# daviidsilvaa/MPI-Model

Hardware: AMD Instinct MI355X
Metric: cell-updates/s (GCUPS) per step + % of HBM roofline (higher is better)
Workload: dtype f64; 1 GPU; c3: 32768x32768 fp64 global, row slabs (BASELINE configs[2]); ranks=1, rows_per_gpu=32768, n_attr=1, parallelism=row-slab x1, rows_per_wave=2548

## Files before the change

mpi-model_amd/csrc/mm_engine.hip:

```cpp
#include <rccl/rccl.h>

#include <algorithm>
#include <cmath>
#include <cstdio>
#include <cstdlib>
#include <cstring>
#include <map>
#include <string>
#include <vector>

#include "../../include/mpimodel.h"
#include "mm_inst.hpp"
#include "mm_plan.hpp"

static_assert(MM_FIELD_MAX_STEPS == mm::kFieldMaxSteps, "include/mpimodel.h: MM_FIELD_MAX_STEPS");

namespace {

thread_local std::string g_last_error;

int fail(int code, const std::string& msg) {
    g_last_error = msg;
    return code;
}
// ... 212 lines not shown
}

constexpr int kPermIdentity = 0 | 1 << 2 | 2 << 4 | 3 << 6;

int relabel(const mm_engine* e, mm::PassArgs& A) {
    if (e->na == 1) return kPermIdentity;
    const Pass& p = e->passes[0];
    int perm[mm::kMaxAttr], inv[mm::kMaxAttr], n = 0;
    for (int a = 0; a < e->na; ++a)
        if ((p.diffuse_mask >> a) & 1) perm[n++] = a;
    const int nd = n;
    for (int a = 0; a < e->na; ++a)
        if (!((p.diffuse_mask >> a) & 1)) perm[n++] = a;
    int code = 0;
    for (int i = 0; i < e->na; ++i) {
        inv[perm[i]] = i;
        code |= perm[i] << (2 * i);
        A.in[i] = e->buf[e->cur][perm[i]];
        A.out[i] = e->buf[e->cur ^ 1][perm[i]];
        A.drate[i] = p.drate[perm[i]];
    }
    A.diffuse_mask = (1 << nd) - 1;
    for (size_t t = 0; t < p.pre.size(); ++t) {
        A.pre_a[t] = (signed char)inv[p.pre[t].a];
        A.pre_b[t] = (signed char)(p.pre[t].b < 0 ? -1 : inv[p.pre[t].b]);
    }
    for (size_t t = 0; t < p.post.size(); ++t) {
        A.post_a[t] = (signed char)inv[p.post[t].a];
        A.post_b[t] = (signed char)(p.post[t].b < 0 ? -1 : inv[p.post[t].b]);
    }
    return code;
}

int slots_per_cu(mm_engine* e, mm::Kernel kernel, int k, bool red) {
    const bool wide = kernel == mm::kWide;
    const mm::KernelInst* inst = mm::find_inst(
        inst_key(e, kernel, k, wide ? (e->na > 1 ? 2 : 4) : 2, true, red, e->variant & 1));
    if (!inst) return 1;
    int& s = e->slots[inst];
    if (!s) s = std::max(1, mm::inst_blocks_per_cu(*inst) * (wide ? 1 : mm::kWavesPerBlock));
    return s;
}

bool field_halo(const mm_engine* e) { return e->d.nranks > 1 || e->d.halo_mode != MM_HALO_NONE; }

void sync_program(mm_engine* e) {
    mm::PlanIn& pin = e->pin;
    pin.n_passes = (int)e->passes.size();
    const Pass* p = pin.n_passes == 1 ? &e->passes[0] : nullptr;
    pin.diffuse_mask = p ? p->diffuse_mask : 0;
    pin.chains = p && !(p->pre.empty() && p->post.empty());
    pin.ring = wring(e);
    pin.field = false;
    for (const Pass& q : e->passes) pin.field = pin.field || q.field_mask != 0;
    bool eight = e->na > 1;
    for (const Pass& q : e->passes)
        eight = eight || !q.pre.empty() || !q.post.empty() || q.field_mask != 0;
    pin.knobs.th = eight ? 8 : e->th_env;
    const bool alone = e->na == 1 && p && p->field_mask == 1 && p->diffuse_mask == 0 && !pin.chains;
    pin.field_k = alone ? mm::field_k_for(pin, field_halo(e)) : 0;
}

int halo_rccl(mm_engine* e, int depth) {
    const int r = e->d.rank, n = e->d.nranks;
    const long long P = e->pitch, h = e->d.h;
    const size_t cnt = (size_t)(depth * P);
    MM_NCCL(ncclGroupStart());
    for (int a = 0; a < e->na; ++a) {
        double* b = e->buf[e->cur][a];
        if (e->self_halo) {
// ... 29 lines not shown
    if (rccl_halo(e)) MM_TRY(halo_rccl(e, depth));
    MM_HIP(hipStreamWaitEvent(e->s_comm, e->ev_comp_mark, 0));
    return MM_OK;
}

int unsplit_halo(mm_engine* e, int depth) {
    if (!rccl_halo(e)) return MM_OK;
    MM_HIP(hipEventRecord(e->ev_ready, e->s_comp));
    MM_HIP(hipStreamWaitEvent(e->s_comm, e->ev_ready, 0));
    MM_TRY(halo_rccl(e, depth));
    MM_HIP(hipEventRecord(e->ev_halo, e->s_comm));
    MM_HIP(hipStreamWaitEvent(e->s_comp, e->ev_halo, 0));
    return MM_OK;
}

int launch(mm_engine* e, const mm::PassLaunches& pl, bool red, const mm::PassArgs& A, hipStream_t s,
           bool border) {
    const int nt = border ? 0 : e->variant;
    if (pl.kern.kernel != mm::kOneStep)
        MM_HIP(mm::launch_kstep(
            inst_key(e, pl.kern.kernel, pl.depth, pl.kern.cols, A.seg != 0, red, nt & 1), A, s));
    else if (A.field_mask)
        MM_HIP(mm::launch_field(e->na, red, A, s, nt));
    else
        MM_HIP(mm::launch_pass(e->na, red, A, s, e->variant));
    return MM_OK;
}

void set_launch(mm::PassArgs& A, const mm::Launch& l) {
    A.ra0 = (int)l.lo, A.ra1 = (int)l.hi, A.rb0 = (int)l.lo2, A.rb1 = (int)l.hi2;
    A.seg = l.seg, A.th = l.th, A.th_edge = l.th_edge, A.xcd_remap = l.xcd_remap;
    A.nstrips = l.nstrips;
    A.waves_a = l.waves_a, A.waves_total = l.waves_total, A.partial_base = l.partial_base;
}

int enqueue_pass(mm_engine* e, const Pass& p, int k, int mask, bool time_it, bool prime = false) {
    const bool red = mask != 0;
    const mm::PassLaunches pl = mm::pass_launches(e->pin, k, red);
    mm::PassArgs A;
    fill_args(e, p, A);
    const int perm = pl.kern.kernel == mm::kWide ? relabel(e, A) : kPermIdentity;
    mm::PassArgs B = A;
    set_launch(A, pl.interior);
    set_launch(B, pl.border);
    if (prime) {
        A.waves_total = B.waves_total = 0;
        A.waves_a = B.waves_a = -1;
        MM_TRY(launch(e, pl, red, A, e->s_comp, false));
        if (pl.split) MM_TRY(launch(e, pl, red, B, e->s_comm, true));
        return MM_OK;
    }
    if (pl.split)
        MM_TRY(split_comp(e));
    else if (e->pin.split)
        MM_TRY(unsplit_halo(e, pl.depth));
    hipEvent_t t0 = nullptr, t1 = nullptr;
    if (time_it) {
        t0 = next_event(e);
        t1 = next_event(e);
        if (!t0 || !t1) return fail(MM_ERR_HIP, "hipEventCreate failed");
        e->ev_bytes.resize(e->ev_used / 2);
        e->ev_bytes.back() = (16.0 * e->na + 8.0 * __builtin_popcount((unsigned)p.field_mask)) *
                             (double)(pl.interior.hi - pl.interior.lo) * (double)e->d.W;
        MM_HIP(hipEventRecord(t0, e->s_comp));
    }
    MM_TRY(launch(e, pl, red, A, e->s_comp, false));
// ... 215 lines not shown
}

int mm_engine_create(const mm_desc* desc, mm_engine** out) {
    if (!desc || !out) return fail(MM_ERR_INVALID, "mm_engine_create: null argument");
    *out = nullptr;
    const mm_desc& d = *desc;
    if (d.H <= 0 || d.W <= 0 || d.h <= 0 || d.x_init < 0 || d.x_init + d.h > d.H)
        return fail(MM_ERR_INVALID, "mm_engine_create: slab outside the grid");
    if (d.n_attr < 1 || d.n_attr > mm::kMaxAttr)
        return fail(MM_ERR_INVALID, "mm_engine_create: n_attr must be 1..4");
    if (d.nranks < 1 || d.rank < 0 || d.rank >= d.nranks)
        return fail(MM_ERR_INVALID, "mm_engine_create: bad rank/nranks");
    if (d.nranks == 1 && (d.x_init != 0 || d.h != d.H))
        return fail(MM_ERR_INVALID, "mm_engine_create: a single slab must own the whole grid");
    if (d.halo_mode == MM_HALO_RCCL && !d.comm_id)
        return fail(MM_ERR_INVALID, "mm_engine_create: MM_HALO_RCCL needs comm_id");
    if (d.nranks > 1 && d.halo_mode == MM_HALO_NONE)
        return fail(MM_ERR_INVALID, "mm_engine_create: nranks > 1 needs a halo mode");
    if (d.W > (1LL << 30) || d.h > (1LL << 30))
        return fail(MM_ERR_INVALID, "mm_engine_create: slab too large");

    mm_engine* e = new mm_engine();
    e->d = d;
    e->na = d.n_attr;
    e->pitch = (d.W + mm::kStripCols - 1) / mm::kStripCols * mm::kStripCols;
    e->rows_alloc = d.h + 2 * mm::kGhost;
    mm::PlanIn& pin = e->pin;
    pin.H = d.H, pin.W = d.W, pin.h = d.h, pin.x_init = d.x_init, pin.nranks = d.nranks;
    pin.pitch = e->pitch, pin.n_attr = d.n_attr;
    pin.min_rows = std::min<long long>(d.h, d.H / d.nranks);
    pin.knobs = mm::read_knobs([](const char* name) -> const char* { return std::getenv(name); });
    e->th_env = pin.knobs.th;
    pin.slots = [e](mm::Kernel kernel, int k, bool red) { return slots_per_cu(e, kernel, k, red); };
    e->variant = mm::kernel_variant(pin);

    auto cleanup = [&](int rc) {
        mm_engine_destroy(e);
        return rc;
    };
    hipError_t he = hipSetDevice(d.device);
    if (he != hipSuccess) return cleanup(fail(MM_ERR_HIP, std::string("hipSetDevice: ") + hipGetErrorString(he)));
    he = hipDeviceGetAttribute(&e->pin.ncu, hipDeviceAttributeMultiprocessorCount, d.device);
    if (he != hipSuccess || e->pin.ncu <= 0) e->pin.ncu = 256;

    const size_t per = (size_t)e->rows_alloc * (size_t)e->pitch;
    const size_t per_al = (per + 31) / 32 * 32;
    e->bytes = sizeof(double) * per_al * 2 * (size_t)e->na;
    if (hipStreamCreateWithFlags(&e->s_comp, hipStreamNonBlocking) != hipSuccess ||
        hipStreamCreateWithFlags(&e->s_comm, hipStreamNonBlocking) != hipSuccess ||
        hipEventCreateWithFlags(&e->ev_ready, hipEventDisableTiming) != hipSuccess ||
        hipEventCreateWithFlags(&e->ev_halo, hipEventDisableTiming) != hipSuccess ||
        hipEventCreateWithFlags(&e->ev_comp_mark, hipEventDisableTiming) != hipSuccess ||
        hipEventCreateWithFlags(&e->ev_comm_done, hipEventDisableTiming) != hipSuccess)
        return cleanup(fail(MM_ERR_HIP, "stream/event creation failed"));

    he = hipMalloc(&e->base, e->bytes);
    if (he != hipSuccess) return cleanup(fail(MM_ERR_NOMEM, std::string("hipMalloc: ") + hipGetErrorString(he)));
    he = hipMemsetAsync(e->base, 0, e->bytes, e->s_comp);
    if (he != hipSuccess) return cleanup(fail(MM_ERR_HIP, std::string("hipMemsetAsync: ") + hipGetErrorString(he)));
    for (int k = 0; k < 2; ++k)
        for (int a = 0; a < e->na; ++a)
            e->buf[k][a] = e->base + per_al * (size_t)(k * e->na + a) + mm::kGhost * e->pitch;

    int rc = ensure_partials(e);
    if (rc != MM_OK) return cleanup(rc);
    e->hist_cap = 1 << 12;
// ... 561 lines not shown
```

mpi-model_amd/csrc/mm_geom.hpp:

```cpp
#pragma once

namespace mm {

constexpr int kMaxAttr = 4;
constexpr int kMaxChain = 4;
constexpr int kStripCols = 128;
constexpr int kWavesPerBlock = 4;
constexpr int kBlock = 64 * kWavesPerBlock;
constexpr int kMaxSteps = 10;
constexpr int kMaxWide = 20;
constexpr int kGhost = kMaxWide;
constexpr int kBorderRows = 4;
constexpr int kSegPrefetch1 = 8;
constexpr int kWide20Waves = 4;
constexpr int kWideRingWaves = 4;

constexpr int span3(long long n, long long i) {
    return (i >= 0 && i < n) ? 1 + (i > 0) + (i < n - 1) : 0;
}

inline int passk_out_cols(int k) { return kStripCols - 4 * ((k + 1) / 2); }

inline int passk_max_steps(int na) { return na == 1 ? kMaxSteps : 2; }

inline long long passk_max_rows(int k, long long pitch) {
    return (1LL << 31) / (pitch * 8) - (3 * k + 2 * kSegPrefetch1 + 8);
}

constexpr int kFieldMaxSteps = 4;
constexpr int kFieldPrefetch = 8;
constexpr int field_ring(int k) {
    return (kFieldPrefetch + 2 * (k - 1) + kFieldPrefetch - 1) / kFieldPrefetch * kFieldPrefetch;
}

inline long long fieldk_max_rows(int k, long long pitch) {
    return (1LL << 31) / (pitch * 8) - (3 * k + 2 * field_ring(k) + 8);
}

inline bool wide_has(int k, int c, int na) {
    if (na > 1) return na == 4 && c == 2 && (k == 4 || k == 8);
    return c == 4 && (k == 4 || k == 8 || k == 12 || k == 16 || k == 20);
}

inline int wide_out_cols(int k, int c) {
    return 64 * c - 2 * c * ((k + c - 1) / c);
}

inline int wide_waves_per_block(int k, int c, int na, bool ring) {
    if (!wide_has(k, c, na)) return 0;
    if (na > 1 && k == 8 && ring) return kWideRingWaves;
    if (na == 1 && k == 20) return kWide20Waves;
    return 4;
}

}
```

mpi-model_amd/csrc/mm_inst.hpp:

```cpp
#pragma once

#include <algorithm>

#include "mm_internal.hpp"

namespace mm {

struct KernelInst {
    const void* fn;
    int threads;
};

template <auto Kern, int Threads>
const KernelInst* inst_of() {
    static const KernelInst inst{reinterpret_cast<const void*>(Kern), Threads};
    return &inst;
}

inline hipError_t launch_inst(const KernelInst& k, long long blocks, const PassArgs& a,
                              hipStream_t s) {
    void* argv[] = {const_cast<PassArgs*>(&a)};
    (void)hipGetLastError();
    (void)hipLaunchKernel(k.fn, dim3((unsigned)blocks), dim3((unsigned)k.threads), argv, 0, s);
    return hipGetLastError();
// ... 6 lines not shown
        return 0;
    }
    const int regs = (fa.numRegs + 7) / 8 * 8;
    const int waves_per_simd = regs > 0 ? std::min(8, 512 / regs) : 8;
    int blocks = waves_per_simd * 4 / (k.threads / 64);
    if (fa.sharedSizeBytes > 0) blocks = std::min(blocks, (int)(160 * 1024 / fa.sharedSizeBytes));
    return blocks;
}

enum InstFamily { kInstPassK, kInstWide, kInstFieldK };
struct InstKey {
    InstFamily family;
    int k;
    int cols;
    int na;
    bool seg;
    bool red;
    bool nt;
    bool ring;
    bool post;
    int nd;
};

using InstLookup = const KernelInst* (*)(const InstKey&);
#define MM_INST_DECL(name) const KernelInst* name(const InstKey& q);
MM_INST_DECL(passk_inst_k1) MM_INST_DECL(passk_inst_k2) MM_INST_DECL(passk_inst_k3)
MM_INST_DECL(passk_inst_k4) MM_INST_DECL(passk_inst_k5) MM_INST_DECL(passk_inst_k6)
MM_INST_DECL(passk_inst_k7) MM_INST_DECL(passk_inst_k8) MM_INST_DECL(passk_inst_k9)
MM_INST_DECL(passk_inst_k10)
MM_INST_DECL(wide_inst_k4) MM_INST_DECL(wide_inst_k8) MM_INST_DECL(wide_inst_k12)
MM_INST_DECL(wide_inst_k16) MM_INST_DECL(wide_inst_k20)
MM_INST_DECL(wide_inst_k20_r0_n0) MM_INST_DECL(wide_inst_k20_r0_n1)
MM_INST_DECL(wide_inst_k20_r1_n0) MM_INST_DECL(wide_inst_k20_r1_n1)
MM_INST_DECL(widea_inst_k4) MM_INST_DECL(widear_inst_k8)
MM_INST_DECL(widea8_inst_n1_p0) MM_INST_DECL(widea8_inst_n1_p1)
MM_INST_DECL(widea8_inst_n2_p0) MM_INST_DECL(widea8_inst_n2_p1)
MM_INST_DECL(widea8_inst_n3_p0) MM_INST_DECL(widea8_inst_n3_p1)
MM_INST_DECL(widea8_inst_n4_p0) MM_INST_DECL(widea8_inst_n4_p1)
MM_INST_DECL(fieldk_inst_k2) MM_INST_DECL(fieldk_inst_k3) MM_INST_DECL(fieldk_inst_k4)
#undef MM_INST_DECL

const KernelInst* find_inst(const InstKey& q);
hipError_t launch_kstep(const InstKey& q, const PassArgs& a, hipStream_t s);

}
```

mpi-model_amd/csrc/mm_internal.hpp:

```cpp
#pragma once

#include <hip/hip_runtime.h>

#include "mm_geom.hpp"

namespace mm {

struct PassArgs {
    const double* in[kMaxAttr];
    double* out[kMaxAttr];
    long long H, W, x_init, pitch;
    int ra0, ra1, rb0, rb1;
    int th;
    int nstrips;
    long long waves_a;
    long long waves_total;
    int diffuse_mask;
    int npre, npost;
    double drate[kMaxAttr];
    signed char pre_a[kMaxChain], pre_b[kMaxChain];
    signed char post_a[kMaxChain], post_b[kMaxChain];
    double pre_r[kMaxChain], post_r[kMaxChain];
    double* partials;
    long long partial_base;
    int xcd_remap;
    int seg;
    int th_edge;
    const double* field[kMaxAttr];
    int field_mask;
};

hipError_t launch_pass(int na, bool reduce, const PassArgs& a, hipStream_t s, int variant);
hipError_t launch_field(int na, bool reduce, const PassArgs& a, hipStream_t s, int variant);
hipError_t launch_finalize_levels(const double* partials, long long n, int k, int na, int mask,
                                  double* hist, unsigned long long* hist_n, long long cap,
                                  hipStream_t s, int perm);
hipError_t launch_fill(double* buf, long long pitch, long long H, long long W, long long x_init,
                       long long h, int mode, double value, unsigned long long seed, hipStream_t s);
hipError_t launch_point(double* buf, long long pitch, long long H, long long W, long long x_init,
                        long long h, long long sx, long long sy, double captured, double rate,
                        hipStream_t s);
hipError_t launch_finalize(const double* partials, long long n, int na, double* hist,
                           unsigned long long* hist_n, long long cap, hipStream_t s,
                           int entries = 1);
hipError_t launch_slab_sum(const double* buf, long long pitch, long long W, long long h,
                           double* partials, long long nblocks, double* out_sum, hipStream_t s);

}
```

mpi-model_amd/csrc/mm_kernels_k.hip:

```cpp
#include "mm_wide.hpp"

namespace mm {

namespace {

__global__ __launch_bounds__(256) void mm_level_sums_kernel(const double* partials, long long n,
                                                            int k, int na, int mask,
                                                            double* hist,
                                                            unsigned long long* hist_n,
                                                            long long cap, int perm) {
    __shared__ double red[256];
    const int e = (int)blockIdx.x / na, a = (int)blockIdx.x % na;
    int j = 0;
    for (int c = -1; j < k; ++j)
        if (((mask >> j) & 1) && ++c == e) break;
    double s = 0.0;
    for (long long i = threadIdx.x; i < n; i += 256) s = s + partials[(i * k + j) * na + a];
    red[threadIdx.x] = s;
    __syncthreads();
    for (int m = 128; m >= 1; m >>= 1) {
        if ((int)threadIdx.x < m) red[threadIdx.x] = red[threadIdx.x] + red[threadIdx.x + m];
        __syncthreads();
    }
    if (threadIdx.x == 0) {
// ... 2 lines not shown
        const long long idx = (long long)slot + e;
        if (idx < cap) hist[idx * na + ((perm >> (2 * a)) & 3)] = red[0];
        const unsigned long long done = __hip_atomic_fetch_add(
            hist_n + 1, 1ull, __ATOMIC_ACQ_REL, __HIP_MEMORY_SCOPE_AGENT);
        if (done == (unsigned long long)gridDim.x - 1) {
            const int entries = __builtin_popcount((unsigned)mask);
            __hip_atomic_store(hist_n, slot + (unsigned long long)entries, __ATOMIC_RELAXED,
                               __HIP_MEMORY_SCOPE_AGENT);
            __hip_atomic_store(hist_n + 1, 0ull, __ATOMIC_RELAXED, __HIP_MEMORY_SCOPE_AGENT);
        }
    }
}

}

hipError_t launch_finalize_levels(const double* partials, long long n, int k, int na, int mask,
                                  double* hist, unsigned long long* hist_n, long long cap,
                                  hipStream_t s, int perm) {
    const int entries = __builtin_popcount((unsigned)mask);
    if (entries == 0) return hipSuccess;
    hipLaunchKernelGGL(mm_level_sums_kernel, dim3((unsigned)(entries * na)), dim3(256), 0, s,
                       partials, n, k, na, mask, hist, hist_n, cap, perm);
    return hipGetLastError();
}

static_assert(seg_prefetch<1>() == kSegPrefetch1,
              "mm_geom.hpp: passk_max_rows counts MM_SEG_U1 rows");

const KernelInst* find_inst(const InstKey& q) {
    static constexpr InstLookup kUnits[] = {
        passk_inst_k1,     passk_inst_k2,     passk_inst_k3,     passk_inst_k4,
        passk_inst_k5,     passk_inst_k6,     passk_inst_k7,     passk_inst_k8,
        passk_inst_k9,     passk_inst_k10,    wide_inst_k4,      wide_inst_k8,
        wide_inst_k12,     wide_inst_k16,     wide_inst_k20,     widea_inst_k4,
        widear_inst_k8,    widea8_inst_n1_p0, widea8_inst_n1_p1, widea8_inst_n2_p0,
        widea8_inst_n2_p1, widea8_inst_n3_p0, widea8_inst_n3_p1, widea8_inst_n4_p0,
        widea8_inst_n4_p1, fieldk_inst_k2,    fieldk_inst_k3,    fieldk_inst_k4};
    for (InstLookup unit : kUnits)
        if (const KernelInst* inst = unit(q)) return inst;
    return nullptr;
}

hipError_t launch_kstep(const InstKey& q, const PassArgs& a, hipStream_t s) {
    if (a.waves_total <= 0 && a.waves_a >= 0) return hipSuccess;
    const KernelInst* inst = find_inst(q);
    if (!inst) return hipErrorInvalidValue;
    long long blocks = std::max<long long>(a.waves_total, 1);
    if (q.family == kInstFieldK) {
        if (!a.field[0] || a.field_mask != 1) return hipErrorInvalidValue;
        if (!q.seg && a.th != kBorderRows) return hipErrorInvalidValue;
        blocks = std::max<long long>(1, (a.waves_total + kWavesPerBlock - 1) / kWavesPerBlock);
    } else if (q.family == kInstPassK) {
        if (!q.seg && a.th != kBorderRows) return hipErrorInvalidValue;
        blocks = std::max<long long>(1, (a.waves_total + kWavesPerBlock - 1) / kWavesPerBlock);
        if (a.xcd_remap) blocks = (blocks + 7) / 8 * 8;
    }
    return launch_inst(*inst, blocks, a, s);
}

}
```

mpi-model_amd/csrc/mm_plan.cpp:

```cpp
#include "mm_plan.hpp"

#include <algorithm>
#include <cmath>
#include <cstdlib>

namespace mm {

namespace {

constexpr double kAny = 1e300;

struct KnobRow {
    const char* name;
    char type;
    double lo, hi;
    void (*set)(Knobs&, double);
};

const KnobRow kKnobRows[] = {
    {"MM_GRAPH", 'i', -kAny, kAny, [](Knobs& k, double v) { k.graphs_ok = v != 0; }},
    {"MM_GRAPH_MIN_STEPS", 'i', 1, 256, [](Knobs& k, double v) { k.graph_min = (long long)v; }},
    {"MM_GRAPH_MAX_LAUNCHES", 'i', 1, 4096, [](Knobs& k, double v) { k.graph_max = (long long)v; }},
    {"MM_ROWS_PER_WAVE", 'i', 8, 32, [](Knobs& k, double v) { if (v == 8 || v == 16 || v == 32) k.th = (int)v; }},
    {"MM_FUSE", 'i', -kAny, kAny, [](Knobs& k, double v) { k.passk = k.passk && v != 0; }},
    {"MM_PASSK", 'i', -kAny, kAny, [](Knobs& k, double v) { k.passk = k.passk && v != 0; }},
    {"MM_WIDE", 'i', -kAny, kAny, [](Knobs& k, double v) { k.wide = v != 0 ? 1 : 0; }},
    {"MM_STEPS_PER_PASS", 'i', 1, kAny,
     [](Knobs& k, double d) {
         const int v = (int)std::min(d, 1e9);
         if (v <= kMaxSteps || (k.wide != 0 && (wide_has(v, 4, 1) || wide_has(v, 2, 4)))) k.kpass = v;
         k.kpass_multi = std::min(v, 2);
     }},
    {"MM_PASS_PLAN", 'i', -kAny, kAny, [](Knobs& k, double v) { k.plan = v != 0; }},
    {"MM_SEG_WAVES", 'd', 0, kAny, [](Knobs& k, double v) { k.seg_waves = v; }},
    {"MM_SEG_EDGE", 'd', 0, 1, [](Knobs& k, double v) { k.seg_edge = v; }},
    {"MM_XCD_REMAP", 'i', -kAny, kAny, [](Knobs& k, double v) { k.xcd = v != 0; }},
    {"MM_BORDER_SEGMENTS", 'i', -kAny, kAny, [](Knobs& k, double v) { k.border_segments = v != 0; }},
    {"MM_CHAIN_RING", 'i', -kAny, kAny, [](Knobs& k, double v) { k.ring_ok = v != 0; }},
    {"MM_SYNC_SPIN", 'i', -kAny, kAny, [](Knobs& k, double v) { k.sync_spin = v != 0; }},
    {"MM_SELF_HALO", 'i', -kAny, kAny, [](Knobs& k, double v) { k.self_halo = v != 0; }},
    {"MM_KERNEL_VARIANT", 'i', 0, kAny, [](Knobs& k, double v) { k.variant = (int)std::min(v, 1e9); }},
    {"MM_FIELD_STEPS", 'i', 0, kFieldMaxSteps, [](Knobs& k, double v) { k.field_steps = (int)v; }},
    {"MM_FIELD_HALO", 'i', 1, kFieldMaxSteps, [](Knobs& k, double v) { k.field_halo = (int)v; }},
};

}

Knobs read_knobs(const std::function<const char*(const char*)>& get) {
    Knobs k;
    for (const KnobRow& r : kKnobRows) {
        const char* s = get(r.name);
        if (!s) continue;
        const double v = r.type == 'i' ? (double)std::atoll(s) : std::atof(s);
        if ((r.type == 'i' ? v >= r.lo : v > r.lo) && v <= r.hi) r.set(k, v);
    }
    return k;
}

namespace {

constexpr double kWideCells = 268435456.0;
constexpr double kWideSmallCells = 33554432.0;
constexpr int kWideSmallAuto = 8;
constexpr double kWideSplitCells = 134217728.0;
constexpr int kWideAuto = 20;
constexpr int kWideAutoMulti = 8;

double slab_cells(const PlanIn& in) { return (double)in.min_rows * (double)in.W; }

int wcols(const PlanIn& in) { return in.n_attr > 1 ? 2 : 4; }

bool wide_big(const PlanIn& in) {
    return in.knobs.wide > 0 || slab_cells(in) >= kWideCells ||
           (in.knobs.wide < 0 && in.n_attr == 1 && slab_cells(in) >= kWideSplitCells);
}

// ... 88 lines not shown
static_assert(kFieldAutoCells >= 65536.0 && kFieldAutoSteps <= kFieldMaxSteps, "auto rule");
constexpr double kFieldAutoCellsHalo = 4194304.0;
static_assert(kFieldAutoCellsHalo >= kFieldAutoCells, "a halo never lowers the auto threshold");

}

int field_steps_for(const PlanIn& in) {
    const int k = in.knobs.field_steps;
    if (!in.knobs.passk || k == 1 || in.pitch <= 0 || fieldk_max_rows(kFieldMaxSteps, in.pitch) < 64)
        return 0;
    if (k >= 2) return std::min(k, kFieldMaxSteps);
    return (double)in.h * (double)in.W >= kFieldAutoCells ? kFieldAutoSteps : 0;
}

int field_k_for(const PlanIn& in, bool halo) {
    if (!halo) return field_steps_for(in);
    PlanIn thin = in;
    thin.h = in.min_rows;
    int k = field_steps_for(thin);
    if (in.knobs.field_steps == 0 && slab_cells(in) < kFieldAutoCellsHalo) k = 0;
    k = (int)std::min<long long>(std::min(k, in.knobs.field_halo), in.min_rows);
    return k >= 2 ? k : 0;
}

bool kstep_ok(const PlanIn& in) { return fieldk_on(in) || passk_ok(in); }

bool passk_ok(const PlanIn& in) {
    if (!in.knobs.passk || in.n_passes != 1 || in.field) return false;
    if (passk_max_rows(kMaxSteps, in.pitch) < 64) return false;
    if (in.n_attr == 1) return in.diffuse_mask == 1 && !in.chains;
    return true;
}

KernelChoice kernel_for(const PlanIn& in, int k) {
    if (fieldk_on(in) && k >= 2) return {kFieldK, 2, ceil_div(in.W, passk_out_cols(k))};
    if (!passk_ok(in)) return {kOneStep, 1, 0};
    if (use_wide(in, k)) return {kWide, wcols(in), ceil_div(in.W, wide_out_cols(k, wcols(in)))};
    return {kPassK, 2, ceil_div(in.W, passk_out_cols(k))};
}

int steps_per_launch(const PlanIn& in) {
    if (fieldk_on(in)) return in.field_k;
    return passk_ok(in) ? passk_steps(in) : 1;
}

int next_pass_len(const PlanIn& in, long long n) {
    if (fieldk_on(in)) return (int)ceil_div(n, ceil_div(n, in.field_k));
    if (!passk_ok(in)) return 1;
    const Knobs& kn = in.knobs;
    const int kp = passk_steps(in);
    if (wide_on(in)) {
        if (in.n_attr == 1 && kn.kpass == 0 && kn.plan && wide_big(in)) {
            int cap = kMaxWide;
            if (in.nranks > 1) cap = (int)std::min<long long>(cap, in.min_rows);
            return wide_plan_first(in, n, cap);
        }
        long long k = std::min<long long>(n, kp);
        while (k > 1 && !pass_len_ok(in, k)) --k;
        return (int)std::max<long long>(1, k);
    }
    long long best_p = ceil_div(n, kp);
    const bool big = slab_cells(in) >= kWideCells && ceil_div(in.W, passk_out_cols(kMaxSteps)) >= 256;
    if (kn.plan && kn.kpass == 0 && in.n_attr == 1 && big && n > kp) {
        long long kx = passk_max_steps(1);
        if (in.nranks > 1) kx = std::min<long long>(kx, in.min_rows);
        double best = 1e300;
        const long long p_max = best_p;
        for (long long p = ceil_div(n, kx); p <= p_max; ++p) {
            const long long q = n / p, r = n % p;
            const double t = (double)r * pass_cost((int)q + 1) + (double)(p - r) * pass_cost((int)q);
            if (t < best * (1.0 - 1e-9)) {
// ... 22 lines not shown
        16, kernel == kFieldK ? fieldk_max_rows(k, in.pitch) : passk_max_rows(k, in.pitch));
    const double edge = seg_edge_of(in, kernel, k);
    const double units = ns < 3 ? (double)ns / edge : (double)(ns - 2) + 2.0 / edge;
    auto even_rows = [&](long long rr) { return std::min(maxr & ~1LL, rr + (rr & 1)); };
    auto re_of = [&](long long rr) {
        return even_rows(std::min(maxr, std::max<long long>(8, (long long)((double)rr * edge))));
    };
    auto plan = [&](double sw) {
        const long long want = std::max<long long>(1, (long long)(sw * in.ncu * slots));
        long long r = (long long)std::ceil((double)std::max<long long>(n, 1) * units / (double)want);
        r = std::min(std::max<long long>(r, 16), maxr);
        while (r < maxr && seg_wave_count(n, ns, r, re_of(r)) > want) r += std::max<long long>(1, r / 64);
        return even_rows(std::min(r, maxr));
    };
    long long r;
    if (in.knobs.seg_waves > 0.0) {
        r = plan(in.knobs.seg_waves);
    } else if (kernel == kWide) {
        double sw = 4.0;
        r = plan(sw);
        while (sw > 1.0 && r < 20LL * k) {
            sw -= 1.0;
            r = plan(sw);
        }
    } else {
        r = plan(4.0);
        if (r < 256) r = plan(2.0);
    }
    const long long re = re_of(r);
    return {(int)r, (int)re, seg_wave_count(n, ns, r, re)};
}

Segments segments(const PlanIn& in, int k, bool red, long long lo, long long hi) {
    const KernelChoice kc = kernel_for(in, k);
    return segments(in, kc.kernel, k, std::max(1, in.slots(kc.kernel, k, red)), hi - lo, kc.strips);
}

PassLaunches pass_launches(const PlanIn& in, int k, bool red) {
    PassLaunches p{};
    p.kern = kernel_for(in, k);
    const Kernel kernel = p.kern.kernel;
    const long long h = in.h;
    const int ns = kernel == kOneStep ? (int)(in.pitch / kStripCols) : (int)p.kern.strips;
    p.depth = kernel == kOneStep ? 1 : k;
    p.split = in.split && h >= 2 * p.depth + 1;
    auto blocks = [&](long long lo, long long hi, long long lo2, long long hi2, int th) {
        Launch l;
        l.lo = lo, l.hi = hi, l.lo2 = lo2, l.hi2 = hi2, l.th = th, l.nstrips = ns;
        l.waves_a = waves_for(ns, hi - lo, th);
        l.waves_total = l.waves_a + waves_for(ns, hi2 - lo2, th);
        return l;
    };
    auto segs = [&](long long lo, long long hi) {
        const Segments s = segments(in, k, red, lo, hi);
        Launch l;
        l.lo = lo, l.hi = hi, l.seg = 1, l.th = s.th, l.th_edge = s.th_edge, l.nstrips = ns;
        l.waves_a = l.waves_total = s.count;
        return l;
    };
    long long T = p.split ? p.depth : 0;
    if (p.split && kernel == kWide && in.knobs.border_segments)
        T = std::min<long long>(std::max<long long>(segs(0, h).th, p.depth), h / 2);
    p.interior = kernel == kOneStep ? blocks(T, h - T, 0, 0, in.knobs.th) : segs(T, h - T);
    if (kernel == kPassK) p.interior.xcd_remap = in.knobs.xcd;
    if (p.split) {
        if (kernel == kWide) {
            p.border = blocks(0, T, h - T, h, (int)T);
            p.border.seg = 1, p.border.th_edge = (int)T;
            p.border.waves_a = seg_wave_count(T, ns, T, T);
            p.border.waves_total = 2 * p.border.waves_a;
        } else {
            p.border = blocks(0, T, h - T, h, kernel == kOneStep ? 1 : kBorderRows);
        }
        p.border.partial_base = p.interior.waves_total;
    }
    p.total = p.interior.waves_total + p.border.waves_total;
    return p;
}

SlabPlan slab_plan(const PlanIn& in) {
    const int spl = steps_per_launch(in);
    const KernelChoice kc = kernel_for(in, spl);
    if (kc.kernel == kOneStep)
        return {kOneStep, spl, in.knobs.th, waves_for(in.pitch / kStripCols, in.h, in.knobs.th), 0};
    const Segments s = segments(in, spl, false, 0, in.h);
    const int per = kc.kernel == kWide ? wide_waves_per_block(spl, kc.cols, in.n_attr, in.ring) : 1;
    return {kc.kernel, spl, s.th, s.count * per, std::max(1, in.slots(kc.kernel, spl, false)) * per};
}

long long graph_per(const PlanIn& in, long long nsteps, long long reduce_every, bool any) {
    auto gcd = [](long long a, long long b) {
        while (b) {
            const long long t = a % b;
            a = b;
            b = t;
        }
        return a;
    };
    const long long unit = steps_per_launch(in);
    const long long flips = kstep_ok(in) ? 1 : (long long)in.n_passes;
    long long len = unit * ((flips % 2) ? 2 : 1);
    if (reduce_every > 0) len = len / gcd(len, reduce_every) * reduce_every;
    if (len > 256 || nsteps < len || (!in.knobs.graphs_ok && !any)) return 0;
    long long per = len;
    while (per < in.knobs.graph_min && per * 2 <= nsteps) per *= 2;
    if (nsteps % per != 0 && nsteps <= 64 * unit) per = nsteps;
    const long long base = reduce_every > 0 ? unit / gcd(unit, reduce_every) * reduce_every : unit;
    if (nsteps % base == 0) {
        const long long m = nsteps / base, per_block = base / unit * flips;
        for (long long d = std::min(m, in.knobs.graph_max / per_block); d * base > per; --d)
            if (m % d == 0) {
                per = d * base;
                break;
            }
    }
    return per;
}

long long partials_need(const PlanIn& in) {
// ... 14 lines not shown
```

mpi-model_amd/csrc/mm_plan.hpp:

```cpp
#pragma once

#include <functional>
#include <vector>

#include "mm_geom.hpp"

namespace mm {

struct Knobs {
    bool graphs_ok = true;
    long long graph_min = 16;
    long long graph_max = 128;
    int th = 8;
    bool passk = true;
    int wide = -1;
    int kpass = 0;
    int kpass_multi = 2;
    bool plan = true;
    double seg_waves = 0.0;
    double seg_edge = 0.0;
    bool border_segments = true;
    int xcd = 0;
    bool ring_ok = true;
    bool sync_spin = true;
    bool self_halo = false;
    int variant = -1;
    int field_steps = 0;
    int field_halo = 1;
};
Knobs read_knobs(const std::function<const char*(const char*)>& get);

enum Kernel { kOneStep = 0, kPassK = 2, kWide = 3, kFieldK = 4 };

struct PlanIn {
    long long H = 0, W = 0, h = 0, x_init = 0;
    int nranks = 1;
    long long min_rows = 0;
    long long pitch = 0;
    int n_attr = 1;
    bool split = false;
    int n_passes = 0;
    int diffuse_mask = 0;
    bool chains = false;
    bool ring = false;
    bool field = false;
    int field_k = 0;
    Knobs knobs;
    int ncu = 0;
    std::function<int(Kernel, int k, bool red)> slots;
};

struct KernelChoice {
    Kernel kernel;
    int cols;
    long long strips;
};

struct Segments {
    int th, th_edge;
    long long count;
};

struct Launch {
    long long lo = 0, hi = 0, lo2 = 0, hi2 = 0;
    int seg = 0, th = 0, th_edge = 0, xcd_remap = 0, nstrips = 0;
    long long waves_a = 0, waves_total = 0, partial_base = 0;
};

struct PassLaunches {
    KernelChoice kern;
    int depth;
    bool split;
    Launch interior, border;
    long long total;
};

bool passk_ok(const PlanIn& in);
int field_steps_for(const PlanIn& in);
int field_k_for(const PlanIn& in, bool halo);
bool kstep_ok(const PlanIn& in);
KernelChoice kernel_for(const PlanIn& in, int k);
int steps_per_launch(const PlanIn& in);
int next_pass_len(const PlanIn& in, long long n);
std::vector<int> pass_lengths(const PlanIn& in, long long n);
long long seg_wave_count(long long n, long long ns, long long r, long long re);
Segments segments(const PlanIn& in, Kernel kernel, int k, int slots, long long n, long long ns);
Segments segments(const PlanIn& in, int k, bool red, long long lo, long long hi);
PassLaunches pass_launches(const PlanIn& in, int k, bool red);
struct SlabPlan {
    Kernel kernel;
    int steps_per_launch, rows_per_wave;
    long long waves_per_pass;
    int seg_waves_per_cu;
};
SlabPlan slab_plan(const PlanIn& in);
long long graph_per(const PlanIn& in, long long nsteps, long long reduce_every, bool any = false);
long long partials_need(const PlanIn& in);
int kernel_variant(const PlanIn& in);

}
```

mpi-model_amd/csrc/mm_wide.hpp:

```cpp
#pragma once

#include "mm_passk.hpp"

#ifndef MM_WIDE_GEN_ROW
#define MM_WIDE_GEN_ROW 1
#endif

namespace mm {

namespace {

#ifndef MM_WIDE_U
#define MM_WIDE_U 4
#endif
#ifndef MM_WIDE_B
#define MM_WIDE_B 4
#endif
#ifndef MM_WIDE_MIN_WAVES
#define MM_WIDE_MIN_WAVES 2
#endif
#ifndef MM_WIDE_PRO_MID
#define MM_WIDE_PRO_MID 1
#endif
#ifndef MM_WIDE_ASC
// ... 583 lines not shown
        }
    }
    wave_groups<C, NA, KW, P, U, B, RED, NT, kBodyGen, ROLE, PP>(x, st, (int)f1, iend);
    if (RED) {
        const bool lane_owns = x.c.own[0];
#pragma unroll
        for (int q = 0; q < KW; ++q) {
#pragma unroll
            for (int a = 0; a < NA; ++a)
                carry[q][a] = carry[q][a] + wave_sum(lane_owns ? st.acc[q][a] : 0.0);
        }
    }
}

template <int C, int NA, int KW, int P, int U, int B, bool RED, int NT, int MID>
__device__ __forceinline__ void wave_dispatch(const WCtx<C, NA>& x, int iend,
                                              double (&carry)[KW][NA]) {
    constexpr bool kMidPar = ((KW | WGeom<KW, P, B>::D) & 1) != 0;
    if (P == 1)
        wave_run<C, NA, KW, P, U, B, RED, NT, kRoleOnly, MID, 0>(x, iend, carry);
    else if (x.p == 0)
        wave_run<C, NA, KW, P, U, B, RED, NT, kRoleFirst, MID, 0>(x, iend, carry);
    else if (x.p == P - 1)
        wave_run<C, NA, KW, P, U, B, RED, NT, kRoleLast, MID, (P - 1) & 1>(x, iend, carry);
    else if (kMidPar && (x.p & 1))
        wave_run<C, NA, KW, P, U, B, RED, NT, kRoleMid, MID, 1>(x, iend, carry);
    else
        wave_run<C, NA, KW, P, U, B, RED, NT, kRoleMid, MID, 0>(x, iend, carry);
}

template <int C, int NA, int KW, int P, int U, int B, bool RED, int NT>
__device__ __forceinline__ void wide_segment(const PassArgs& A, dv2* lds, int p, int lane,
                                             int strip, int rA, int rB,
                                             double (&carry)[KW][NA]) {
    using G = WGeom<KW, P, B>;
    constexpr int K = G::K;
    constexpr int LH = (K + C - 1) / C;
    constexpr int OC = 64 * C - 2 * C * LH;
    constexpr int RW = 32 * C * NA;
    WCtx<C, NA> x;
    const int sh = (int)((A.x_init + rA - K) & 1);
    x.rA = rA - sh;
    x.oA = rA;
    x.rB = rB;
    const long long W = A.W;
    const long long c0 = (long long)strip * OC - C * LH;
    const long long y0 = c0 + C * lane;
    const bool in_row = y0 >= 0 && y0 < A.pitch;
    const bool store_lane = lane >= LH && lane < 64 - LH && y0 < W;
    x.rowb = (unsigned)(A.pitch * 8);
    x.voff = (in_row ? (unsigned)(y0 * 8) : kOOB) - (unsigned)sh * x.rowb;
    x.soff = store_lane ? (unsigned)(y0 * 8) : kOOB;
    x.c.H = A.H;
#pragma unroll
    for (int k = 0; k < C; ++k) {
        x.c.sy[k] = span3(W, y0 + k);
        x.c.own[k] = store_lane && y0 + k < W;
        x.c.ownw[k] = x.c.own[k] ? 1.0 : 0.0;
    }
    x.p = p;
    x.lane = lane;
    x.start = p * G::D;
    x.dmask = MM_ND ? (1 << MM_ND) - 1 : A.diffuse_mask;
    x.g0 = A.x_init + x.rA - K;
#pragma unroll
    for (int a = 0; a < NA; ++a) {
        x.r8[a] = A.drate[a] * 0.125;
        x.in[a] = rows_rsrc(A.in[a] + (long long)(rA - K) * A.pitch, rB - rA + 2 * K, A.pitch);
        x.out[a] = rows_rsrc(A.out[a] + (long long)rA * A.pitch, rB - rA, A.pitch);
    }
    x.none = rows_rsrc(A.out[0], 0, A.pitch);
    x.lds_in = p > 0 ? lds + (p - 1) * G::RL * RW : lds;
    x.lds_out = p < P - 1 ? lds + p * G::RL * RW : lds;
    x.A = &A;
    if (MM_CHAIN_ASM) {
#pragma unroll
        for (int t = 0; t < kMaxChain; ++t) {
            const bool pu = t < A.npre, qu = t < A.npost;
            x.pia[t] = pu ? 2 * A.pre_a[t] : 8;
// ... 23 lines not shown
    const int lane = threadIdx.x & 63;
    const int p = __builtin_amdgcn_readfirstlane(threadIdx.x >> 6);
    const long long blk = blockIdx.x;
    if (blk >= A.waves_total) return;
    int rlo, rhi;
    long long w = blk;
    if (w < A.waves_a) {
        rlo = A.ra0;
        rhi = A.ra1;
    } else {
        w -= A.waves_a;
        rlo = A.rb0;
        rhi = A.rb1;
    }
    int strip, rA, rB;
    seg_map(w, rlo, rhi, A.nstrips, A.th, A.th_edge, strip, rA, rB);
    double carry[KW][NA];
#pragma unroll
    for (int q = 0; q < KW; ++q) {
#pragma unroll
        for (int a = 0; a < NA; ++a) carry[q][a] = 0.0;
    }
    wide_segment<C, NA, KW, P, U, B, RED, NT>(A, lds, p, lane, strip, rA, rB, carry);
    if (RED && lane == 0) {
#pragma unroll
        for (int q = 0; q < KW; ++q) {
#pragma unroll
            for (int a = 0; a < NA; ++a)
                A.partials[((A.partial_base + blk) * K + p * KW + q) * NA + a] = carry[q][a];
        }
    }
}

template <int C, int NA, int KW, int P>
bool wide_key(const InstKey& q) {
    return q.family == kInstWide && q.k == KW * P && q.cols == C && q.na == NA && q.seg;
}

template <int C, int NA, int KW, int P, int MW, bool RED, int NT>
const KernelInst* wide_inst_v() {
    return inst_of<mm_wide_kernel<C, NA, KW, P, MW, MM_WIDE_U, MM_WIDE_B, RED, NT>, 64 * P>();
}

template <int C, int NA, int KW, int P, int MW>
const KernelInst* wide_inst(const InstKey& q) {
    if (!wide_key<C, NA, KW, P>(q)) return nullptr;
    if (q.nt)
        return q.red ? wide_inst_v<C, NA, KW, P, MW, true, 1>()
                     : wide_inst_v<C, NA, KW, P, MW, false, 1>();
    return q.red ? wide_inst_v<C, NA, KW, P, MW, true, 0>()
                 : wide_inst_v<C, NA, KW, P, MW, false, 0>();
}

}

}
```

mpi-model_amd/csrc/mm_wide_k16.hip:

```cpp
#ifndef MM_WIDE_U
#define MM_WIDE_U 2
#endif
#include "mm_wide.hpp"

namespace mm {

const KernelInst* wide_inst_k16(const InstKey& q) {
    return wide_inst<4, 1, 4, 4, MM_WIDE_MIN_WAVES>(q);
}

}
```

Baseline: 3550 GCUPS.

## Add 6-column-per-lane wide K=20 kernel with fast interior path

Adds a wide K=20 kernel variant in which interior row bands use 6 columns per lane and a simplified fast path (no span/ownership per column, single attribute, no reduction). Top and bottom border bands and the leftover column strips keep the 4-column path. A new planner decides the band and strip layout and work partitioning, and the new kernel is selected automatically for large single-rank, single-attribute slabs. Wider lanes cut the halo overhead per output column and the per-column bookkeeping, at the cost of more registers and lower occupancy. The K=16 instantiation is also split into separate compilation parts.

```diff
diff --git a/mpi-model_amd/csrc/mm_engine.hip b/mpi-model_amd/csrc/mm_engine.hip
--- a/mpi-model_amd/csrc/mm_engine.hip
+++ b/mpi-model_amd/csrc/mm_engine.hip
@@ -268,10 +268,11 @@
     return code;
 }
 
-int slots_per_cu(mm_engine* e, mm::Kernel kernel, int k, bool red) {
+int slots_per_cu(mm_engine* e, mm::Kernel kernel, int k, bool red, int cols = 0) {
     const bool wide = kernel == mm::kWide;
-    const mm::KernelInst* inst = mm::find_inst(
-        inst_key(e, kernel, k, wide ? (e->na > 1 ? 2 : 4) : 2, true, red, e->variant & 1));
+    if (!cols) cols = wide ? (e->na > 1 ? 2 : 4) : 2;
+    const mm::KernelInst* inst =
+        mm::find_inst(inst_key(e, kernel, k, cols, true, red, e->variant & 1));
     if (!inst) return 1;
     int& s = e->slots[inst];
     if (!s) s = std::max(1, mm::inst_blocks_per_cu(*inst) * (wide ? 1 : mm::kWavesPerBlock));
@@ -367,6 +368,10 @@
     A.seg = l.seg, A.th = l.th, A.th_edge = l.th_edge, A.xcd_remap = l.xcd_remap;
     A.nstrips = l.nstrips;
     A.waves_a = l.waves_a, A.waves_total = l.waves_total, A.partial_base = l.partial_base;
+    const mm::Wide6& w = l.c6;
+    A.c6_top = w.top, A.c6_bot = w.bot, A.c6_col = w.col, A.c6_rcol = w.rcol;
+    A.c6_strips = w.strips, A.c6_rstrips = w.rstrips, A.c6_th = w.th;
+    A.c6_band0 = w.band0, A.c6_band1 = w.band1, A.c6_frame = w.frame;
 }
 
 int enqueue_pass(mm_engine* e, const Pass& p, int k, int mask, bool time_it, bool prime = false) {
@@ -648,6 +653,7 @@
     pin.knobs = mm::read_knobs([](const char* name) -> const char* { return std::getenv(name); });
     e->th_env = pin.knobs.th;
     pin.slots = [e](mm::Kernel kernel, int k, bool red) { return slots_per_cu(e, kernel, k, red); };
+    pin.slots6 = [e](int k) { return slots_per_cu(e, mm::kWide, k, false, mm::kWide6Cols); };
     e->variant = mm::kernel_variant(pin);
 
     auto cleanup = [&](int rc) {
diff --git a/mpi-model_amd/csrc/mm_geom.hpp b/mpi-model_amd/csrc/mm_geom.hpp
--- a/mpi-model_amd/csrc/mm_geom.hpp
+++ b/mpi-model_amd/csrc/mm_geom.hpp
@@ -14,6 +14,7 @@
 constexpr int kSegPrefetch1 = 8;
 constexpr int kWide20Waves = 4;
 constexpr int kWideRingWaves = 4;
+constexpr int kWide6Cols = 6;
 
 constexpr int span3(long long n, long long i) {
     return (i >= 0 && i < n) ? 1 + (i > 0) + (i < n - 1) : 0;
@@ -46,6 +47,18 @@
     return 64 * c - 2 * c * ((k + c - 1) / c);
 }
 
+struct Wide6Cols {
+    int col, rcol, strips, rstrips;
+};
+inline Wide6Cols wide6_cols(long long W) {
+    const int o4 = wide_out_cols(kMaxWide, 4), o6 = wide_out_cols(kMaxWide, kWide6Cols);
+    const int halo = kWide6Cols * ((kMaxWide + kWide6Cols - 1) / kWide6Cols);
+    const long long room = W - o4 - (halo + 1);
+    const int n = room >= o6 && W < (1LL << 30) ? (int)(room / o6) : 0;
+    const int rcol = o4 + n * o6;
+    return {o4, rcol, n, n ? (int)((W - rcol + o4 - 1) / o4) : 0};
+}
+
 inline int wide_waves_per_block(int k, int c, int na, bool ring) {
     if (!wide_has(k, c, na)) return 0;
     if (na > 1 && k == 8 && ring) return kWideRingWaves;
diff --git a/mpi-model_amd/csrc/mm_inst.hpp b/mpi-model_amd/csrc/mm_inst.hpp
--- a/mpi-model_amd/csrc/mm_inst.hpp
+++ b/mpi-model_amd/csrc/mm_inst.hpp
@@ -62,6 +62,9 @@
 MM_INST_DECL(wide_inst_k16) MM_INST_DECL(wide_inst_k20)
 MM_INST_DECL(wide_inst_k20_r0_n0) MM_INST_DECL(wide_inst_k20_r0_n1)
 MM_INST_DECL(wide_inst_k20_r1_n0) MM_INST_DECL(wide_inst_k20_r1_n1)
+MM_INST_DECL(wide_inst_k16_r0_n0) MM_INST_DECL(wide_inst_k16_r0_n1)
+MM_INST_DECL(wide_inst_k16_r1_n0) MM_INST_DECL(wide_inst_k16_r1_n1)
+MM_INST_DECL(wide6_inst_k20)
 MM_INST_DECL(widea_inst_k4) MM_INST_DECL(widear_inst_k8)
 MM_INST_DECL(widea8_inst_n1_p0) MM_INST_DECL(widea8_inst_n1_p1)
 MM_INST_DECL(widea8_inst_n2_p0) MM_INST_DECL(widea8_inst_n2_p1)
diff --git a/mpi-model_amd/csrc/mm_internal.hpp b/mpi-model_amd/csrc/mm_internal.hpp
--- a/mpi-model_amd/csrc/mm_internal.hpp
+++ b/mpi-model_amd/csrc/mm_internal.hpp
@@ -28,6 +28,11 @@
     int th_edge;
     const double* field[kMaxAttr];
     int field_mask;
+    int c6_top, c6_bot;
+    int c6_col, c6_rcol;
+    int c6_strips, c6_rstrips;
+    int c6_th;
+    long long c6_band0, c6_band1, c6_frame;
 };
 
 hipError_t launch_pass(int na, bool reduce, const PassArgs& a, hipStream_t s, int variant);
diff --git a/mpi-model_amd/csrc/mm_kernels_k.hip b/mpi-model_amd/csrc/mm_kernels_k.hip
--- a/mpi-model_amd/csrc/mm_kernels_k.hip
+++ b/mpi-model_amd/csrc/mm_kernels_k.hip
@@ -58,7 +58,8 @@
         passk_inst_k1,     passk_inst_k2,     passk_inst_k3,     passk_inst_k4,
         passk_inst_k5,     passk_inst_k6,     passk_inst_k7,     passk_inst_k8,
         passk_inst_k9,     passk_inst_k10,    wide_inst_k4,      wide_inst_k8,
-        wide_inst_k12,     wide_inst_k16,     wide_inst_k20,     widea_inst_k4,
+        wide_inst_k12,     wide_inst_k16,     wide_inst_k20,     wide6_inst_k20,
+        widea_inst_k4,
         widear_inst_k8,    widea8_inst_n1_p0, widea8_inst_n1_p1, widea8_inst_n2_p0,
         widea8_inst_n2_p1, widea8_inst_n3_p0, widea8_inst_n3_p1, widea8_inst_n4_p0,
         widea8_inst_n4_p1, fieldk_inst_k2,    fieldk_inst_k3,    fieldk_inst_k4};
diff --git a/mpi-model_amd/csrc/mm_plan.cpp b/mpi-model_amd/csrc/mm_plan.cpp
--- a/mpi-model_amd/csrc/mm_plan.cpp
+++ b/mpi-model_amd/csrc/mm_plan.cpp
@@ -42,6 +42,7 @@
     {"MM_KERNEL_VARIANT", 'i', 0, kAny, [](Knobs& k, double v) { k.variant = (int)std::min(v, 1e9); }},
     {"MM_FIELD_STEPS", 'i', 0, kFieldMaxSteps, [](Knobs& k, double v) { k.field_steps = (int)v; }},
     {"MM_FIELD_HALO", 'i', 1, kFieldMaxSteps, [](Knobs& k, double v) { k.field_halo = (int)v; }},
+    {"MM_WIDE_COLS", 'i', 4, kWide6Cols, [](Knobs& k, double v) { if (v != 5) k.wide_cols = (int)v; }},
 };
 
 }
@@ -196,11 +197,31 @@
     return true;
 }
 
-KernelChoice kernel_for(const PlanIn& in, int k) {
+bool wide6_on(const PlanIn& in, int k, bool red) {
+    if (!in.slots6 || in.knobs.wide_cols == 4 || k != kMaxWide || red || in.n_attr != 1 || in.split ||
+        in.nranks != 1 || in.x_init != 0 || in.h != in.H || !use_wide(in, k))
+        return false;
+    if (wide6_cols(in.W).strips == 0) return false;
+    return in.knobs.wide_cols == kWide6Cols || slab_cells(in) >= kWideSplitCells;
+}
+
+namespace {
+
+KernelChoice kernel4_for(const PlanIn& in, int k) {
     if (fieldk_on(in) && k >= 2) return {kFieldK, 2, ceil_div(in.W, passk_out_cols(k))};
     if (!passk_ok(in)) return {kOneStep, 1, 0};
     if (use_wide(in, k)) return {kWide, wcols(in), ceil_div(in.W, wide_out_cols(k, wcols(in)))};
     return {kPassK, 2, ceil_div(in.W, passk_out_cols(k))};
+}
+
+}
+
+KernelChoice kernel_for(const PlanIn& in, int k, bool red) {
+    if (wide6_on(in, k, red)) {
+        const Wide6Cols c = wide6_cols(in.W);
+        return {kWide, kWide6Cols, 1 + c.strips + c.rstrips};
+    }
+    return kernel4_for(in, k);
 }
 
 int steps_per_launch(const PlanIn& in) {
@@ -289,13 +310,54 @@
 }
 
 Segments segments(const PlanIn& in, int k, bool red, long long lo, long long hi) {
-    const KernelChoice kc = kernel_for(in, k);
+    const KernelChoice kc = kernel4_for(in, k);
     return segments(in, kc.kernel, k, std::max(1, in.slots(kc.kernel, k, red)), hi - lo, kc.strips);
+}
+
+namespace {
+
+int slots6_of(const PlanIn& in, int k) { return std::max(1, in.slots6(k)); }
+
+Launch wide6_launch(const PlanIn& in, int k) {
+    const Wide6Cols c = wide6_cols(in.W);
+    const long long h = in.h;
+    Launch l;
+    l.lo = 0, l.hi = h, l.seg = 1;
+    l.nstrips = (int)ceil_div(in.W, wide_out_cols(k, 4));
+    Wide6& w = l.c6;
+    w.col = c.col, w.rcol = c.rcol, w.strips = c.strips, w.rstrips = c.rstrips;
+    w.top = (int)std::min<long long>(k + 2, h);
+    w.bot = (int)std::max<long long>(w.top, (h - k - 2) & ~1LL);
+    w.band0 = l.nstrips;
+    w.band1 = w.band0 + (w.bot < h ? l.nstrips : 0);
+    w.frame = w.band1;
+    l.waves_total = w.band1;
+    const long long n = w.bot - w.top;
+    if (n > 0) {
+        const long long ns = 1 + c.rstrips + c.strips;
+        const Segments s = segments(in, kWide, k, slots6_of(in, k), n, ns);
+        l.th = l.th_edge = w.th = s.th;
+        const long long per = ceil_div(n, s.th);
+        w.frame = w.band1 + (1 + c.rstrips) * per;
+        l.waves_total = w.frame + c.strips * per;
+    } else {
+        l.th = l.th_edge = w.th = 2;
+    }
+    l.waves_a = l.waves_total;
+    return l;
+}
+
 }
 
 PassLaunches pass_launches(const PlanIn& in, int k, bool red) {
     PassLaunches p{};
-    p.kern = kernel_for(in, k);
+    p.kern = kernel_for(in, k, red);
+    if (p.kern.cols == kWide6Cols && p.kern.kernel == kWide) {
+        p.depth = k;
+        p.interior = wide6_launch(in, k);
+        p.total = p.interior.waves_total;
+        return p;
+    }
     const Kernel kernel = p.kern.kernel;
     const long long h = in.h;
     const int ns = kernel == kOneStep ? (int)(in.pitch / kStripCols) : (int)p.kern.strips;
@@ -340,8 +402,12 @@
     const KernelChoice kc = kernel_for(in, spl);
     if (kc.kernel == kOneStep)
         return {kOneStep, spl, in.knobs.th, waves_for(in.pitch / kStripCols, in.h, in.knobs.th), 0};
+    if (kc.cols == kWide6Cols && kc.kernel == kWide) {
+        const Launch l = wide6_launch(in, spl);
+        return {kWide, spl, l.th, l.waves_total * kWide20Waves, slots6_of(in, spl) * kWide20Waves};
+    }
     const Segments s = segments(in, spl, false, 0, in.h);
-    const int per = kc.kernel == kWide ? wide_waves_per_block(spl, kc.cols, in.n_attr, in.ring) : 1;
+    const int per =kc.kernel == kWide ? wide_waves_per_block(spl, kc.cols, in.n_attr, in.ring) : 1;
     return {kc.kernel, spl, s.th, s.count * per, std::max(1, in.slots(kc.kernel, spl, false)) * per};
 }
 
diff --git a/mpi-model_amd/csrc/mm_plan.hpp b/mpi-model_amd/csrc/mm_plan.hpp
--- a/mpi-model_amd/csrc/mm_plan.hpp
+++ b/mpi-model_amd/csrc/mm_plan.hpp
@@ -27,6 +27,7 @@
     int variant = -1;
     int field_steps = 0;
     int field_halo = 1;
+    int wide_cols = 0;
 };
 Knobs read_knobs(const std::function<const char*(const char*)>& get);
 
@@ -48,6 +49,7 @@
     Knobs knobs;
     int ncu = 0;
     std::function<int(Kernel, int k, bool red)> slots;
+    std::function<int(int k)> slots6;
 };
 
 struct KernelChoice {
@@ -61,10 +63,16 @@
     long long count;
 };
 
+struct Wide6 {
+    int top = 0, bot = 0, col = 0, rcol = 0, strips = 0, rstrips = 0, th = 0;
+    long long band0 = 0, band1 = 0, frame = 0;
+};
+
 struct Launch {
     long long lo = 0, hi = 0, lo2 = 0, hi2 = 0;
     int seg = 0, th = 0, th_edge = 0, xcd_remap = 0, nstrips = 0;
     long long waves_a = 0, waves_total = 0, partial_base = 0;
+    Wide6 c6;
 };
 
 struct PassLaunches {
@@ -79,7 +87,8 @@
 int field_steps_for(const PlanIn& in);
 int field_k_for(const PlanIn& in, bool halo);
 bool kstep_ok(const PlanIn& in);
-KernelChoice kernel_for(const PlanIn& in, int k);
+KernelChoice kernel_for(const PlanIn& in, int k, bool red = false);
+bool wide6_on(const PlanIn& in, int k, bool red);
 int steps_per_launch(const PlanIn& in);
 int next_pass_len(const PlanIn& in, long long n);
 std::vector<int> pass_lengths(const PlanIn& in, long long n);
diff --git a/mpi-model_amd/csrc/mm_wide.hpp b/mpi-model_amd/csrc/mm_wide.hpp
--- a/mpi-model_amd/csrc/mm_wide.hpp
+++ b/mpi-model_amd/csrc/mm_wide.hpp
@@ -639,7 +639,7 @@
 template <int C, int NA, int KW, int P, int U, int B, bool RED, int NT>
 __device__ __forceinline__ void wide_segment(const PassArgs& A, dv2* lds, int p, int lane,
                                              int strip, int rA, int rB,
-                                             double (&carry)[KW][NA]) {
+                                             double (&carry)[KW][NA], long long col0 = 0) {
     using G = WGeom<KW, P, B>;
     constexpr int K = G::K;
     constexpr int LH = (K + C - 1) / C;
@@ -651,7 +651,7 @@
     x.oA = rA;
     x.rB = rB;
     const long long W = A.W;
-    const long long c0 = (long long)strip * OC - C * LH;
+    const long long c0 = col0 + (long long)strip * OC - C * LH;
     const long long y0 = c0 + C * lane;
     const bool in_row = y0 >= 0 && y0 < A.pitch;
     const bool store_lane = lane >= LH && lane < 64 - LH && y0 < W;
@@ -741,6 +741,94 @@
     }
 }
 
+template <int C, int KW, int P, int U, int B, int NT, int ROLE, int PP>
+__device__ __forceinline__ void wave_run_fast(const WCtx<C, 1>& x, int iend) {
+    static_assert(B % U == 0, "ring slots repeat within a group");
+    WState<C, 1, KW, U> st;
+    const int s = wave_prologue<C, 1, KW, P, U, B, false, NT, ROLE, kBodyFast, PP>(x, st);
+    wave_groups<C, 1, KW, P, U, B, false, NT, kBodyFast, ROLE, PP>(x, st, s, iend);
+}
+
+template <int C, int KW, int P, int U, int B, int NT>
+__device__ __forceinline__ void fast_segment(const PassArgs& A, dv2* lds, int p, int lane,
+                                             long long col, int rA, int rB) {
+    using G = WGeom<KW, P, B>;
+    constexpr int K = G::K;
+    constexpr int LH = (K + C - 1) / C;
+    constexpr int RW = 32 * C;
+    WCtx<C, 1> x;
+    const int sh = (int)((A.x_init + rA - K) & 1);
+    x.rA = rA - sh;
+    x.oA = rA;
+    x.rB = rB;
+    const long long y0 = col - C * LH + C * lane;
+    const bool in_row = y0 >= 0 && y0 + C <= A.pitch;
+    const bool store_lane = lane >= LH && lane < 64 - LH && y0 + C <= A.W;
+    x.rowb = (unsigned)(A.pitch * 8);
+    x.voff = (in_row ? (unsigned)(y0 * 8) : kOOB) - (unsigned)sh * x.rowb;
+    x.soff = store_lane ? (unsigned)(y0 * 8) : kOOB;
+    x.c.H = A.H;
+    x.p = p;
+    x.lane = lane;
+    x.start = p * G::D;
+    x.dmask = 1;
+    x.g0 = A.x_init + x.rA - K;
+    x.r8[0] = A.drate[0] * 0.125;
+    x.in[0] = rows_rsrc(A.in[0] + (long long)(rA - K) * A.pitch, rB - rA + 2 * K, A.pitch);
+    x.out[0] = rows_rsrc(A.out[0] + (long long)rA * A.pitch, rB - rA, A.pitch);
+    x.none = rows_rsrc(A.out[0], 0, A.pitch);
+    x.lds_in = p > 0 ? lds + (p - 1) * G::RL * RW : lds;
+    x.lds_out = p < P - 1 ? lds + p * G::RL * RW : lds;
+    x.A = &A;
+    const int need = (P - 1) * G::D + G::S0 + (x.rB - x.rA);
+    const int iend = (need + G::B - 1) / G::B * G::B;
+    constexpr bool kMidPar = ((KW | G::D) & 1) != 0;
+    if (p == 0)
+        wave_run_fast<C, KW, P, U, B, NT, kRoleFirst, 0>(x, iend);
+    else if (p == P - 1)
+        wave_run_fast<C, KW, P, U, B, NT, kRoleLast, (P - 1) & 1>(x, iend);
+    else if (kMidPar && (p & 1))
+        wave_run_fast<C, KW, P, U, B, NT, kRoleMid, 1>(x, iend);
+    else
+        wave_run_fast<C, KW, P, U, B, NT, kRoleMid, 0>(x, iend);
+}
+
+template <int CF, int CI, int KW, int P, int MW, int U, int B, int NT>
+__global__ __launch_bounds__(64 * P, MW) void mm_wide6_kernel(const PassArgs A) {
+    using G = WGeom<KW, P, B>;
+    constexpr int K = G::K;
+    constexpr int LHI = (K + CI - 1) / CI;
+    constexpr int OCI = 64 * CI - 2 * CI * LHI;
+    static_assert(CI >= CF && CI % 2 == 0 && OCI % 2 == 0, "the LDS rows hold either path's");
+    __shared__ dv2 lds[(P - 1) * G::RL * 32 * CI];
+    const int lane = threadIdx.x & 63;
+    const int p = __builtin_amdgcn_readfirstlane(threadIdx.x >> 6);
+    long long w = blockIdx.x;
+    if (w >= A.waves_total) return;
+    int strip, rA, rB;
+    if (w >= A.c6_frame) {
+        seg_map(w - A.c6_frame, A.c6_top, A.c6_bot, A.c6_strips, A.c6_th, A.c6_th, strip, rA, rB);
+        fast_segment<CI, KW, P, U, B, NT>(A, lds, p, lane, A.c6_col + (long long)strip * OCI, rA,
+                                          rB);
+        return;
+    }
+    double carry[KW][1];
+    long long col0 = 0;
+    if (w < A.c6_band0) {
+        seg_map(w, A.ra0, A.c6_top, A.nstrips, A.c6_top - A.ra0, A.c6_top - A.ra0, strip, rA, rB);
+    } else if (w < A.c6_band1) {
+        seg_map(w - A.c6_band0, A.c6_bot, A.ra1, A.nstrips, A.ra1 - A.c6_bot, A.ra1 - A.c6_bot,
+                strip, rA, rB);
+    } else {
+        seg_map(w - A.c6_band1, A.c6_top, A.c6_bot, 1 + A.c6_rstrips, A.th, A.th, strip, rA, rB);
+        if (strip > 0) {
+            col0 = A.c6_rcol;
+            strip -= 1;
+        }
+    }
+    wide_segment<CF, 1, KW, P, U, B, false, NT>(A, lds, p, lane, strip, rA, rB, carry, col0);
+}
+
 template <int C, int NA, int KW, int P>
 bool wide_key(const InstKey& q) {
     return q.family == kInstWide && q.k == KW * P && q.cols == C && q.na == NA && q.seg;
diff --git a/mpi-model_amd/csrc/mm_wide6_k20.hip b/mpi-model_amd/csrc/mm_wide6_k20.hip
--- /dev/null
+++ b/mpi-model_amd/csrc/mm_wide6_k20.hip
@@ -0,0 +1,26 @@
+#ifndef MM_WIDE_ASC
+#define MM_WIDE_ASC 1
+#endif
+#ifndef MM_WIDE_U
+#define MM_WIDE_U 2
+#endif
+#ifndef MM_K20_KW
+#define MM_K20_KW 5
+#endif
+#include "mm_wide.hpp"
+
+#define MM_K20_P (20 / MM_K20_KW)
+
+namespace mm {
+
+const KernelInst* wide6_inst_k20(const InstKey& q) {
+    if (q.family != kInstWide || q.k != 20 || q.cols != kWide6Cols || q.na != 1 || !q.seg || q.red)
+        return nullptr;
+    return inst_of<mm_wide6_kernel<4, kWide6Cols, MM_K20_KW, MM_K20_P, MM_WIDE_MIN_WAVES,
+                                   MM_WIDE_U, MM_WIDE_B, 1>,
+                   64 * MM_K20_P>();
+}
+
+static_assert(MM_K20_P == kWide20Waves, "mm_geom.hpp: waves per workgroup of the K = 20 instance");
+
+}
diff --git a/mpi-model_amd/csrc/mm_wide_k16.hip b/mpi-model_amd/csrc/mm_wide_k16.hip
--- a/mpi-model_amd/csrc/mm_wide_k16.hip
+++ b/mpi-model_amd/csrc/mm_wide_k16.hip
@@ -3,10 +3,28 @@
 #endif
 #include "mm_wide.hpp"
 
+#define MM_CAT4(a, b, c, d) a##b##c##d
+#define MM_PN(f, r, n) MM_CAT4(f, r, _n, n)
+
 namespace mm {
 
-const KernelInst* wide_inst_k16(const InstKey& q) {
-    return wide_inst<4, 1, 4, 4, MM_WIDE_MIN_WAVES>(q);
+#if defined(MM_PART_RED) && defined(MM_PART_NT)
+
+const KernelInst* MM_PN(wide_inst_k16_r, MM_PART_RED, MM_PART_NT)(const InstKey& q) {
+    if (!wide_key<4, 1, 4, 4>(q) || q.red != (MM_PART_RED != 0) || q.nt != (MM_PART_NT != 0))
+        return nullptr;
+    return wide_inst_v<4, 1, 4, 4, MM_WIDE_MIN_WAVES, MM_PART_RED != 0, MM_PART_NT>();
 }
 
+#else
+
+const KernelInst* wide_inst_k16(const InstKey& q) {
+    for (InstLookup part : {wide_inst_k16_r0_n0, wide_inst_k16_r0_n1, wide_inst_k16_r1_n0,
+                            wide_inst_k16_r1_n1})
+        if (const KernelInst* i = part(q)) return i;
+    return nullptr;
 }
+
+#endif
+
+}
```

New measurement: 3666 GCUPS (median of 6 runs). 1.03x the previous value.
